# bioinfo-pf-curie/mpiBWA

Measured on AMD Instinct MI355X. Metric: Mreads/s (whole node) 2x150 bp PE vs GRCh38-size reference; SAM bit-match, higher is better.
Workload: dtype int32

## Files before the change

mpibwa_amd/csrc/aln_kernel.hip:

```cpp
#include <hip/hip_runtime.h>
#include <algorithm>
#include "device.h"
#include "wave_ext.cuh"

namespace mbw {

#define ALN_WAVES 1
__host__ __device__ inline int aln_zcap(int max_len) { int z = 80 * (max_len + 32); z = (z + 255) & ~255; return z < 12288 ? 12288 : z; }
__host__ __device__ inline int aln_zcap_small(int max_len) { int z = 32 * (max_len + 32); return (z + 255) & ~255; }
#define ALN_MDCAP 768
#define ALN_CIGCAP 96
#define ALN_NEG (-0x40000000)

__device__ __forceinline__ int wave_sum_int(int v)
{
	for (int o = 32; o > 0; o >>= 1) v += __shfl_xor(v, o);
	return v;
}

struct AlnLds {
	int *H, *E, *dummy;
	uint8_t *q, *t, *z, *md;
	uint32_t *cig;
};
#define ALN_PAD 64

__device__ __forceinline__ int put_num(uint8_t *md, int len, int v, int lane)
{
	char buf[12];
	int n = 0;
	if (v == 0) buf[n++] = '0';
	while (v > 0) { buf[n++] = '0' + v % 10; v /= 10; }
	if (lane == 0)
		for (int k = 0; k < n; ++k)
			if (len + k < ALN_MDCAP) md[len + k] = buf[n - 1 - k];
	return len + n;
}

#define ALN_PENDING 2
#define ALN_SLAB 1024u

__device__ __forceinline__ bool aln_invalid(const AlnParams &P, const AlnReq &R, int max_len, int tcap)
{
	const int lq = R.qe - R.qb;
	const long long rlen64 = R.re - R.rb;
	const bool bridging = R.rb < P.l_pac && R.re > P.l_pac;
	return lq <= 0 || rlen64 <= 0 || bridging || lq > max_len || rlen64 > tcap;
}
__device__ __forceinline__ bool aln_same_len(const AlnParams &P, const AlnReq &R, int max_len, int tcap)
{
	return !aln_invalid(P, R, max_len, tcap) && R.re - R.rb == R.qe - R.qb;
}

__global__ void __launch_bounds__(256) aln_classify_kernel(AlnParams P, int n_req, const AlnReq *__restrict__ reqs, int max_len, int tcap,
                                                           int *__restrict__ lists, unsigned long long *counters, int dp_kind)
{
	const int rq = blockIdx.x * 256 + threadIdx.x;
	const bool live = rq < n_req && reqs[rq < n_req ? rq : 0].read >= 0;
	bool nodp = false;
	if (live) nodp = aln_same_len(P, reqs[rq], max_len, tcap);
	const unsigned long long below = (1ull << (threadIdx.x & 63)) - 1;
	for (int pass = 0; pass < 2; ++pass) {
		const bool mine = live && (nodp == (pass == 0));
		const int kind = pass == 0 ? 0 : dp_kind;
		const unsigned long long m = __ballot(mine);
		if (!m) continue;
		unsigned long long base = 0;
		if ((threadIdx.x & 63) == __ffsll((long long)m) - 1) base = atomicAdd(&counters[ALN_CNT + kind], (unsigned long long)__popcll(m));
		base = __shfl(base, __ffsll((long long)m) - 1);
		if (mine) lists[(size_t)kind * n_req + base + __popcll(m & below)] = rq;
	}
}

template <int KIND>
__device__ __forceinline__ void aln_one(int rq, const AlnParams &P, const WxParams &X, int n_req, const AlnReq *__restrict__ reqs,
                                        const uint8_t *__restrict__ seq, const int64_t *__restrict__ off, const uint8_t *__restrict__ pac,
                                        const int *__restrict__ gaptab, AlnHdr *__restrict__ hdr, uint8_t *__restrict__ pool,
                                        unsigned long long *counters, unsigned long long pool_bytes, int max_len, int tcap, int *lists, int dp_kind,
                                        unsigned long long &slab_at, unsigned &slab_left)
{
	extern __shared__ int lds_raw[];
	const int wave = threadIdx.x >> 6, lane = threadIdx.x & 63;
	constexpr bool FAST = KIND == 0;
	const int ALN_ZCAP = KIND == 1 ? aln_zcap_small(max_len) : aln_zcap(max_len);
	AlnLds L;
	if (FAST) {
		const size_t per_wave = (size_t)2 * ((max_len + 3) & ~3) + ALN_MDCAP + 16;
		uint8_t *base = (uint8_t *)lds_raw + (size_t)wave * per_wave;
		L.H = L.E = L.dummy = nullptr; L.z = nullptr;
		L.cig = (uint32_t *)base;
		L.q = base + 16;
		L.t = L.q + ((max_len + 3) & ~3);
		L.md = L.t + ((max_len + 3) & ~3);
	} else {
		const size_t per_wave = (size_t)2 * (max_len + 2 + ALN_PAD) * 4 + 4 + ((max_len + 3) & ~3) + ((tcap + 3) & ~3) + ALN_ZCAP + ALN_MDCAP + ALN_CIGCAP * 4;
		uint8_t *base = (uint8_t *)lds_raw + (size_t)wave * per_wave;
		L.H = (int *)base; L.E = L.H + (max_len + 2 + ALN_PAD);
		L.dummy = L.E + (max_len + 2 + ALN_PAD);
		L.cig = (uint32_t *)(L.dummy + 1);
		L.q = (uint8_t *)(L.cig + ALN_CIGCAP);
		L.t = L.q + ((max_len + 3) & ~3);
		L.z = L.t + ((tcap + 3) & ~3);
		L.md = L.z + ALN_ZCAP;
	}

	AlnReq R = reqs[rq];
	if (KIND != 0) {
		const unsigned long long rb = (unsigned long long)R.rb, re = (unsigned long long)R.re;
		R.rb = (int64_t)((unsigned long long)(unsigned)__builtin_amdgcn_readfirstlane((int)(rb >> 32)) << 32 |
		                 (unsigned)__builtin_amdgcn_readfirstlane((int)rb));
		R.re = (int64_t)((unsigned long long)(unsigned)__builtin_amdgcn_readfirstlane((int)(re >> 32)) << 32 |
		                 (unsigned)__builtin_amdgcn_readfirstlane((int)re));
		R.read = __builtin_amdgcn_readfirstlane(R.read); R.qb = __builtin_amdgcn_readfirstlane(R.qb);
		R.qe = __builtin_amdgcn_readfirstlane(R.qe); R.w2 = __builtin_amdgcn_readfirstlane(R.w2);
		R.truesc = __builtin_amdgcn_readfirstlane(R.truesc);
	}
	const int lq = R.qe - R.qb;
	const long long rlen64 = R.re - R.rb;
	AlnHdr out;
	out.score = 0; out.NM = -1; out.n_cigar = 0; out.md_len = 0; out.pool_off = 0; out.flags = 0;
	const bool invalid = aln_invalid(P, R, max_len, tcap);
	if (invalid) {
		out.flags = 1;
		if (lane == 0) hdr[rq] = out;
		return;
	}
	const int rlen = (int)rlen64;
	const bool rev = R.rb >= P.l_pac;
	const uint8_t *rd = seq + off[R.read];
	for (int j = lane; j < lq; j += 64) L.q[j] = rev ? rd[R.qe - 1 - j] : rd[R.qb + j];
	{
		const long long f0 = rev ? (P.l_pac << 1) - R.re : R.rb;
		for (int i = lane; i < rlen; i += 64) {
			long long f = f0 + i;
			int b = (pac[f >> 2] >> ((~f & 3) << 1)) & 3;
			L.t[i] = rev ? 3 - b : b;
		}
	}
	__builtin_amdgcn_wave_barrier();

	const int oe_del = X.o_del + X.e_del, oe_ins = X.o_ins + X.e_ins, e_del = X.e_del, e_ins = X.e_ins;
	uint32_t plo[5], phi[5];
#pragma unroll
	for (int t = 0; t < 5; ++t) {
		plo[t] = (uint32_t)(uint8_t)X.mat[t * 5] | (uint32_t)(uint8_t)X.mat[t * 5 + 1] << 8 | (uint32_t)(uint8_t)X.mat[t * 5 + 2] << 16 |
		         (uint32_t)(uint8_t)X.mat[t * 5 + 3] << 24;
		phi[t] = (uint32_t)(uint8_t)X.mat[t * 5 + 4];
	}
	const int wmax4 = P.w << 2;
	int w2 = R.w2, last_sc = -(1 << 30), score = 0, n_cig = 0;
	bool fallback = false;
	for (int it = 0;; ) {
		w2 = w2 < wmax4 ? w2 : wmax4;
		if (FAST) {
			int s = 0;
			for (int i = lane; i < lq; i += 64) s += X.mat[L.t[i] * 5 + L.q[i]];
			score = wave_sum_int(s);
			if (w2 != 0) {
				int amax = X.mat[0];
				for (int k = 1; k < 25; ++k) amax = X.mat[k] > amax ? X.mat[k] : amax;
				if (amax <= 0 || (long long)lq * amax - score > (long long)amax + oe_del + oe_ins) {
					if (lane == 0) lists[(size_t)dp_kind * n_req + atomicAdd(&counters[ALN_CNT + dp_kind], 1ull)] = rq;
					return;
				}
			}
			n_cig = 1;
			if (lane == 0) L.cig[0] = (uint32_t)lq << 4;
			__builtin_amdgcn_fence(__ATOMIC_RELEASE, "wavefront");
			__builtin_amdgcn_wave_barrier();
			__builtin_amdgcn_fence(__ATOMIC_ACQUIRE, "wavefront");
			break;
		} else {
			int d_len = rlen - lq; d_len = d_len < 0 ? -d_len : d_len;
			int w = (gaptab[lq] + d_len + 1) >> 1;
			w = w < w2 ? w : w2;
			const int min_w = d_len + 3;
			w = w > min_w ? w : min_w;
			const int n_col = lq < 2 * w + 1 ? lq : 2 * w + 1;
			if ((long long)n_col * rlen > ALN_ZCAP) { fallback = true; break; }
			for (int j = lane; j <= lq; j += 64) {
				L.H[j] = j == 0 ? 0 : (j <= w ? -(X.o_ins + e_ins * j) : ALN_NEG);
				L.E[j] = ALN_NEG;
			}
			__builtin_amdgcn_wave_barrier();
			int vslo = 0, vshi = 0;
			for (int i = 0; i < rlen; ++i) {
				if ((i & 63) == 0) {
					const int tb = i + lane < rlen ? (int)L.t[i + lane] : 4;
					vslo = (int)(tb == 0 ? plo[0] : tb == 1 ? plo[1] : tb == 2 ? plo[2] : tb == 3 ? plo[3] : plo[4]);
					vshi = (int)(tb == 0 ? phi[0] : tb == 1 ? phi[1] : tb == 2 ? phi[2] : tb == 3 ? phi[3] : phi[4]);
				}
				const uint32_t slo = (uint32_t)__builtin_amdgcn_readlane(vslo, i & 63), shi = (uint32_t)__builtin_amdgcn_readlane(vshi, i & 63);
				const int beg = i > w ? i - w : 0, end = i + w + 1 < lq ? i + w + 1 : lq;
				const int hleft0 = beg == 0 ? -(X.o_del + e_del * (i + 1)) : ALN_NEG;
				const int n_row = end - beg;
				int A = ALN_NEG;
				int h_carry = hleft0;
				uint8_t *zi = L.z + (size_t)i * n_col;
				for (int s0 = 0; s0 <= n_row; s0 += 64) {
					const int j = beg + s0 + lane;
					const bool act = s0 + lane < n_row, wr = s0 + lane <= n_row;
					const int diag = L.H[j], e = L.E[j];
					const int qraw = (int)L.q[j];
					const int qb = act ? qraw : 4;
					const int sc = (int)(int8_t)__builtin_amdgcn_perm(shi, slo, (uint32_t)qb | 0x0c0c0c00u);
					const int m = diag + sc;
					const int g = act ? m - oe_ins + j * e_ins : ALN_NEG - (1 << 28);
					const int incl = wx_scan_max(g);
					const int excl = wx_dpp<0x138, 0xf>(ALN_NEG - (1 << 28), incl);
					const int f = max(A, excl + e_ins) - j * e_ins;
					uint8_t d = m >= e ? 0 : 1;
					int h = m >= e ? m : e;
					if (h < f) { d = 2; h = f; }
					int t = m - oe_del;
					int e2 = e - e_del;
					if (e2 > t) d |= 1 << 2; else e2 = t;
					t = m - oe_ins;
					if (f - e_ins > t) d |= 2 << 4;
					const int h_prev = wx_dpp<0x138, 0xf>(h_carry, h);
					(wr ? L.H + j : L.dummy)[0] = h_prev;
					(wr ? L.E + j : L.dummy)[0] = act ? e2 : ALN_NEG;
					(act ? zi + (j - beg) : (uint8_t *)L.dummy)[0] = d;
					A = max(A, __builtin_amdgcn_readlane(incl, 63) + e_ins);
					h_carry = __builtin_amdgcn_readlane(h, 63);
				}
				if (n_row < 0 && lane == 0) { L.H[end] = hleft0; L.E[end] = ALN_NEG; }
				__builtin_amdgcn_wave_barrier();
			}
			score = L.H[lq];
			{
				int which = 0, i = rlen - 1, k = (i + w + 1 < lq ? i + w + 1 : lq) - 1, n = 0;
				uint32_t cur = 0;
				bool ovf = false;
				auto push = [&](uint32_t op, uint32_t len) {
					if (cur && (cur & 0xf) == op) cur += len << 4;
					else {
						if (cur) { if (n < ALN_CIGCAP) { if (lane == 0) L.cig[n] = cur; } else ovf = true; ++n; }
						cur = len << 4 | op;
					}
				};
				while (i >= 0 && k >= 0) {
					which = __builtin_amdgcn_readfirstlane((int)L.z[(size_t)i * n_col + (k - (i > w ? i - w : 0))]) >> (which << 1) & 3;
					if (which == 0) { push(0, 1); --i; --k; }
					else if (which == 1) { push(2, 1); --i; }
					else { push(1, 1); --k; }
				}
				if (i >= 0) push(2, i + 1);
				if (k >= 0) push(1, k + 1);
				if (cur) { if (n < ALN_CIGCAP) { if (lane == 0) L.cig[n] = cur; } else ovf = true; ++n; }
				if (ovf) { fallback = true; break; }
				__builtin_amdgcn_wave_barrier();
				for (int a = lane; a < n / 2; a += 64) { uint32_t x = L.cig[a]; L.cig[a] = L.cig[n - 1 - a]; L.cig[n - 1 - a] = x; }
				__builtin_amdgcn_wave_barrier();
				n_cig = n;
			}
		}
		if (score == last_sc || w2 == wmax4) break;
		last_sc = score;
		w2 <<= 1;
		if (!(++it < 3 && score < R.truesc - P.a)) break;
	}
	if (fallback) {
		if (KIND == 1) {
			if (lane == 0) lists[(size_t)2 * n_req + atomicAdd(&counters[ALN_CNT + 2], 1ull)] = rq;
			return;
		}
		out.flags = 1;
		if (lane == 0) hdr[rq] = out;
		return;
	}
	int md_len = 0, n_mm = 0, n_gap = 0;
	{
		const char *int2base = rev ? "TGCAN" : "ACGTN";
		int x = 0, y = 0, u = 0;
		for (int k = 0; k < n_cig; ++k) {
			const uint32_t c = L.cig[k];
			const int op = c & 0xf, len = (int)(c >> 4);
			if (op == 0) {
				for (int i0 = 0; i0 < len; i0 += 64) {
					const int i = i0 + lane;
					unsigned long long mm = __ballot(i < len && L.q[x + i] != L.t[y + i]);
					int cur = 0;
					const int chunk = len - i0 < 64 ? len - i0 : 64;
					while (mm) {
						const int p = __ffsll((long long)mm) - 1;
						mm &= mm - 1;
						u += p - cur;
						md_len = put_num(L.md, md_len, u, lane);
						if (lane == 0 && md_len < ALN_MDCAP) L.md[md_len] = int2base[L.t[y + i0 + p]];
						++md_len; ++n_mm; u = 0; cur = p + 1;
					}
					u += chunk - cur;
				}
				x += len; y += len;
			} else if (op == 2) {
				if (k > 0 && k < n_cig - 1) {
					md_len = put_num(L.md, md_len, u, lane);
					if (lane == 0 && md_len < ALN_MDCAP) L.md[md_len] = '^';
					++md_len;
					for (int i = lane; i < len; i += 64)
						if (md_len + i < ALN_MDCAP) L.md[md_len + i] = int2base[L.t[y + i]];
					md_len += len;
					u = 0; n_gap += len;
				}
				y += len;
			} else { x += len; n_gap += len; }
		}
		md_len = put_num(L.md, md_len, u, lane);
	}
	if (md_len > ALN_MDCAP) {
		out.flags = 1;
		if (lane == 0) hdr[rq] = out;
		return;
	}
	__builtin_amdgcn_wave_barrier();
	const unsigned need = (unsigned)n_cig * 4 + (((unsigned)md_len + 3) & ~3u);
	unsigned long long at = 0;
	if (need <= slab_left) { at = slab_at; slab_at += need; slab_left -= need; }
	else {
		const unsigned take = need > ALN_SLAB ? need : ALN_SLAB;
		if (lane == 0) at = atomicAdd(&counters[0], (unsigned long long)take);
		at = __shfl(at, 0);
		slab_at = at + need; slab_left = take - need;
	}
	if (at + need > pool_bytes) {
		out.flags = 1;
		if (lane == 0) hdr[rq] = out;
		return;
	}
	uint32_t *pc = (uint32_t *)(pool + at);
	for (int k = lane; k < n_cig; k += 64) pc[k] = L.cig[k];
	uint8_t *pm = pool + at + (size_t)n_cig * 4;
	for (int k = lane; k < md_len; k += 64) pm[k] = L.md[k];
	out.score = score; out.NM = n_mm + n_gap; out.n_cigar = n_cig; out.md_len = md_len; out.pool_off = (uint32_t)(at >> 2); out.flags = 0;
	if (lane == 0) hdr[rq] = out;
}

template <int KIND>
__global__ void __launch_bounds__(64 * ALN_WAVES)
aln_kernel(AlnParams P, WxParams X, int n_req, const AlnReq *__restrict__ reqs, const uint8_t *__restrict__ seq,
           const int64_t *__restrict__ off, const uint8_t *__restrict__ pac, const int *__restrict__ gaptab, AlnHdr *__restrict__ hdr,
           uint8_t *__restrict__ pool, unsigned long long *counters, unsigned long long pool_bytes, int max_len, int tcap, int *lists, int dp_kind)
{
	const int wave = threadIdx.x >> 6;
	const int n = (int)counters[ALN_CNT + KIND];
	const int *mine = lists + (size_t)KIND * n_req;
	unsigned long long slab_at = 0;
	unsigned slab_left = 0;
	for (int k = blockIdx.x * ALN_WAVES + wave; k < n; k += gridDim.x * ALN_WAVES) {
		aln_one<KIND>(KIND != 0 ? __builtin_amdgcn_readfirstlane(mine[k]) : mine[k], P, X, n_req, reqs, seq, off, pac, gaptab, hdr, pool, counters, pool_bytes, max_len, tcap, lists, dp_kind,
		              slab_at, slab_left);
		__builtin_amdgcn_fence(__ATOMIC_RELEASE, "wavefront");
		__builtin_amdgcn_wave_barrier();
		__builtin_amdgcn_fence(__ATOMIC_ACQUIRE, "wavefront");
	}
}

size_t aln_lds_per_block(int max_len, int tcap)
{
	const int ALN_ZCAP = aln_zcap(max_len);
	size_t per_wave = (size_t)2 * (max_len + 2 + ALN_PAD) * 4 + 4 + ((max_len + 3) & ~3) + ((tcap + 3) & ~3) + ALN_ZCAP + ALN_MDCAP + ALN_CIGCAP * 4;
	return per_wave * ALN_WAVES;
}

void launch_aln(void *stream, const AlnParams &P, const ExtParams &ep, int n_req, const AlnReq *d_req, const uint8_t *d_seq,
                const int64_t *d_off, const uint8_t *d_pac, const int *d_gaptab, AlnHdr *d_hdr, uint8_t *d_pool,
                unsigned long long *d_counters, size_t pool_bytes, int max_len, int tcap, int *d_lists, bool wide_only)
{
	if (n_req <= 0) return;
	const WxParams X = wx_params(ep);
	const size_t shmem = aln_lds_per_block(max_len, tcap);
	const size_t shmem_small = shmem - (size_t)(aln_zcap(max_len) - aln_zcap_small(max_len)) * ALN_WAVES;
	const size_t shmem_fast = ((size_t)2 * ((max_len + 3) & ~3) + ALN_MDCAP + 16) * ALN_WAVES;
	if (shmem > 64 * 1024 && hipFuncSetAttribute((const void *)aln_kernel<2>, hipFuncAttributeMaxDynamicSharedMemorySize, (int)shmem) != hipSuccess)
		die("aln_kernel: cannot reserve %zu bytes of LDS", shmem);
	if (shmem_small > 64 * 1024 && hipFuncSetAttribute((const void *)aln_kernel<1>, hipFuncAttributeMaxDynamicSharedMemorySize, (int)shmem_small) != hipSuccess)
		die("aln_kernel: cannot reserve %zu bytes of LDS", shmem_small);
	if (shmem_fast > 64 * 1024) die("aln_kernel: reads of %d bp do not fit the LDS staging buffers", max_len);
	static int s_cus = 0;
	if (!s_cus) {
		int dev = 0;
		hipDeviceProp_t prop;
		if (hipGetDevice(&dev) != hipSuccess || hipGetDeviceProperties(&prop, dev) != hipSuccess) die("aln_kernel: cannot query the device");
		s_cus = prop.multiProcessorCount > 0 ? prop.multiProcessorCount : 256;
	}
	auto grid_for = [&](size_t lds) {
		long long per_cu = (long long)(160 * 1024 / std::max<size_t>(lds, 1));
		per_cu = std::max(1ll, std::min(per_cu, 32ll / ALN_WAVES));
		return dim3((unsigned)std::min<long long>((long long)s_cus * per_cu * 2, ((long long)n_req + ALN_WAVES - 1) / ALN_WAVES));
	};
	const dim3 block(64 * ALN_WAVES);
	hipStream_t st = (hipStream_t)stream;
	hipLaunchKernelGGL(aln_classify_kernel, dim3((n_req + 255) / 256), dim3(256), 0, st, P, n_req, d_req, max_len, tcap, d_lists, d_counters,
	                   wide_only ? 2 : 1);
	hipLaunchKernelGGL(aln_kernel<0>, grid_for(shmem_fast), block, shmem_fast, st, P, X, n_req, d_req, d_seq, d_off, d_pac, d_gaptab, d_hdr, d_pool,
	                   d_counters, (unsigned long long)pool_bytes, max_len, tcap, d_lists, wide_only ? 2 : 1);
	hipLaunchKernelGGL(aln_kernel<1>, grid_for(shmem_small), block, shmem_small, st, P, X, n_req, d_req, d_seq, d_off, d_pac, d_gaptab, d_hdr, d_pool,
	                   d_counters, (unsigned long long)pool_bytes, max_len, tcap, d_lists, wide_only ? 2 : 1);
	hipLaunchKernelGGL(aln_kernel<2>, grid_for(shmem), block, shmem, st, P, X, n_req, d_req, d_seq, d_off, d_pac, d_gaptab, d_hdr, d_pool,
	                   d_counters, (unsigned long long)pool_bytes, max_len, tcap, d_lists, wide_only ? 2 : 1);
	if (hipGetLastError() != hipSuccess) die("aln_kernel: launch failed");
}

}
```

mpibwa_amd/csrc/device.h:

```cpp
#ifndef MBW_DEVICE_H
#define MBW_DEVICE_H
#include "internal.h"
#include <mutex>
#include <vector>

namespace mbw {

struct FmDev {
	const void *blk;
	const void *occ32;
	const void *occ_sb;
	const uint64_t *sa;
	const uint64_t *sa_full;
	uint64_t primary, seq_len;
	uint64_t L2[5];
	int sa_shift;
	const void *p3tab;
	int p3_k;
	const void *kmt;
	int kmt_k;
};

struct DevIndex {
	int device = -1;
// ... 82 lines not shown
struct DevReg {
	int64_t rb, re;
	int32_t qb, qe, rid, score, truesc, w, seedcov, seedlen0;
	float frac_rep;
	int32_t pad;
};
struct C2aParams {
	int64_t l_pac;
	int a, w, pen_clip5, pen_clip3;
	int early;
};
struct C2aUnits {
	int max_units = 0, heavy_t = 0;
	const unsigned int *n_units = nullptr;
	const int *ustart = nullptr;
	const int *unit_rd = nullptr, *unit_av = nullptr;
	const int *clist = nullptr;
	int *c_rabs = nullptr, *c_rcnt = nullptr;
};
struct C2aGroupBufs {
	PinBuf h_heavy, h_hoff, h_nunits;
	DevBuf heavy, hoff, scratch, clist, ustart, unit_rd, unit_av, nunits, c_rabs, c_rcnt;
	void release()
	{
		for (PinBuf *b : {&h_heavy, &h_hoff, &h_nunits}) b->release();
		for (DevBuf *b : {&heavy, &hoff, &scratch, &clist, &ustart, &unit_rd, &unit_av, &nunits, &c_rabs, &c_rcnt}) b->release();
	}
};
C2aUnits c2a_prepare_units(void *stream, C2aGroupBufs &B, int heavy_t, int n, const int *chain_cnt, size_t n_chain_slots, const int *d_chain_beg,
                           const int *d_reg_beg, const DevChain *d_chains, int *d_nregs, void (*wait)(void *stream) = nullptr);
void c2a_launch_order(int n, const int *nseeds, int *order);
void c2a_length_tables(const mem_opt_t *opt, int max_len, std::vector<int> &tab);
void c2a_params(const mem_opt_t *opt, int64_t l_pac, int early, C2aParams &cp, ExtParams &ep);
size_t c2a_groups_scratch_bytes(int n_el);
void launch_c2a_groups(void *stream, int n_el, int n_heavy, const int *d_hoff, const int *d_heavy, const int *d_chain_beg, const int *d_reg_beg,
                       const DevChain *d_chains, void *d_scratch, int *d_clist, int *d_ustart, int *d_unit_rd, int *d_unit_av, unsigned int *d_n_units);
#define C2A_STAT_SLOTS 256
void launch_c2a(void *stream, const C2aParams &P, const ExtParams &ep, int n_reads, const uint8_t *d_seq, const int64_t *d_off,
                const int *d_len, const int *d_chain_beg, const int *d_chain_cnt, const DevChain *d_chains, const DevSeed *d_seeds, unsigned int *d_srt,
                const int *d_reg_beg, DevReg *d_regs, int *d_nregs, const int *d_tab, int tab_stride, const uint8_t *d_pac, unsigned long long *d_counters,
                int max_len, const int *d_order = nullptr, const C2aUnits *units = nullptr );

struct ChainParams {
	int64_t l_pac;
	int w, max_chain_gap, min_chain_weight, min_seed_len, max_chain_extend;
	float mask_level, drop_ratio;
};
ChainParams chain_params(const mem_opt_t *opt, int64_t l_pac);
void contig_table(const bntseq_t *bns, std::vector<int64_t> &ann_off, std::vector<uint8_t> &ann_alt);
void launch_chain(void *stream, const ChainParams &P, int n_reads, const int *d_len, const int *d_nseeds, const int *d_lrep,
                  const int64_t *d_seed_off, const uint64_t *d_sa, const int32_t *d_qbl, const int64_t *d_ann_off, const uint8_t *d_ann_alt,
                  int n_seqs, const int *d_tab, int tab_stride, DevChain *d_chains, DevSeed *d_seeds, unsigned int *d_srt, int *d_nchains,
                  void *d_scratch);
size_t chain_scratch_bytes(int n_reads);

size_t reg_pack_tmp_bytes(int n_reads);
void launch_reg_pack(void *stream, int n_reads, const int *d_reg_beg, const int *d_nregs, int *d_reg_pos, const DevReg *d_regs, DevReg *d_packed,
                     void *d_tmp, size_t tmp_bytes, const C2aUnits *units = nullptr, const int *d_chain_beg = nullptr, const int *d_chain_cnt = nullptr);
struct C2aJob {
	int n_reads = 0, max_len = 0;
	const uint8_t *d_seq = nullptr; const int64_t *d_off = nullptr; const int *d_len = nullptr;
	const int *d_chain_beg = nullptr, *d_chain_cnt = nullptr, *d_reg_beg = nullptr, *d_order = nullptr;
	const DevChain *d_chains = nullptr; const DevSeed *d_seeds = nullptr; unsigned int *d_srt = nullptr;
	const int *d_tab = nullptr; int tab_stride = 0;
	const uint8_t *d_pac = nullptr;
	C2aUnits units;
	DevReg *d_regs = nullptr; int *d_nregs = nullptr;
	unsigned long long *d_stat = nullptr;
	int *d_reg_pos = nullptr; DevReg *d_packed = nullptr; void *d_tmp = nullptr; size_t tmp_bytes = 0;
};
void queue_c2a(void *stream, const mem_opt_t *opt, int64_t l_pac, int early, const C2aJob &J, void *ev_a = nullptr, void *ev_b = nullptr);

struct AlnReq {
	int64_t rb, re;
	int32_t read, qb, qe, w2, truesc, pad;
};
struct AlnHdr {
	int32_t score, NM, n_cigar, md_len;
	uint32_t pool_off;
	int32_t flags;
};
struct AlnParams { int64_t l_pac; int a, w; };
#define ALN_CNT 8
void aln_params(const mem_opt_t *opt, int64_t l_pac, AlnParams &ap, ExtParams &ep);
inline size_t aln_pool_bytes(size_t n_req) { return n_req * 96 + ((size_t)48 << 20); }
void cigar_gap_table(const mem_opt_t *opt, int max_len, std::vector<int> &tab);
size_t aln_lds_per_block(int max_len, int tcap);
void launch_aln(void *stream, const AlnParams &P, const ExtParams &ep, int n_req, const AlnReq *d_req, const uint8_t *d_seq,
                const int64_t *d_off, const uint8_t *d_pac, const int *d_gaptab, AlnHdr *d_hdr, uint8_t *d_pool,
                unsigned long long *d_counters, size_t pool_bytes, int max_len, int tcap, int *d_lists ,
                bool wide_only = false );

struct SamDesc {
	int64_t rb, re;
	int32_t qb, qe;
	int32_t req;
	int32_t rid, flag, mapq, score, sub;
};
#define SAM_XA_SHIFT 16
#define SAM_XA_MASK 15
struct SamParams {
	int64_t l_pac;
	int has_qual, rg_len;
	char rg[256];
};
SamParams sam_params(int64_t l_pac, bool has_qual);
void contig_names(const bntseq_t *bns, std::vector<char> &names, std::vector<int> &name_off);
size_t sam_arena_bytes(int n_reads, int max_len);
struct ChunkDev {
	const uint8_t *d_seq = nullptr; const int64_t *d_off = nullptr; const int *d_len = nullptr; int max_len = 0;
	const uint8_t *d_pac = nullptr; const int *d_gap = nullptr;
	const uint8_t *d_qual = nullptr, *d_names = nullptr; const int *d_noff = nullptr;
	const int64_t *d_ann_off = nullptr; const uint8_t *d_ann_alt = nullptr; const char *d_ann_names = nullptr; const int *d_ann_noff = nullptr;
};
struct AlnSamJob {
	int n_req = 0; const AlnReq *d_req = nullptr; AlnHdr *d_hdr = nullptr; uint8_t *d_pool = nullptr; size_t pool_bytes = 0;
	unsigned long long *d_cnt = nullptr; int *d_lists = nullptr;
	int ends = 2, r0 = 0, n_reads = 0;
	const SamDesc *h_desc = nullptr;
	SamDesc *d_desc = nullptr;
	const int *h_base = nullptr; int *d_base = nullptr;
	uint8_t *d_arena = nullptr; size_t arena_bytes = 0; unsigned long long *d_used = nullptr, *d_ooff = nullptr; int *d_olen = nullptr;
	int grid_blocks = 0;
	int n_multi = 0; const int *d_mlist = nullptr; const uint8_t *d_mlines = nullptr; const SamDesc *d_mdesc = nullptr; const int *d_mbase = nullptr;
};
void queue_aln_sam(void *stream, const mem_opt_t *opt, int64_t l_pac, const ChunkDev &D, const SamParams &sp, const AlnSamJob &J,
                   void *ev_a = nullptr, void *ev_b = nullptr);
void launch_sam_emit(void *stream, const SamParams &P, int n_reads, const SamDesc *d_desc, const int *d_req_base, const AlnReq *d_req, const AlnHdr *d_hdr,
                     const uint8_t *d_pool, const uint8_t *d_seq, const int64_t *d_off, const int *d_len, const uint8_t *d_qual,
                     const uint8_t *d_names, const int *d_name_off, const int64_t *d_ann_off, const char *d_ann_names, const int *d_ann_name_off,
                     uint8_t *d_arena, size_t arena_bytes, unsigned long long *d_arena_used, unsigned long long *d_out_off, int *d_out_len,
                     int grid_blocks = 0);
void launch_sam_emit_se(void *stream, const SamParams &P, int n_reads, const SamDesc *d_desc, const int *d_req_base, const AlnReq *d_req, const AlnHdr *d_hdr,
                        const uint8_t *d_pool, const uint8_t *d_seq, const int64_t *d_off, const int *d_len, const uint8_t *d_qual,
                        const uint8_t *d_names, const int *d_name_off, const int64_t *d_ann_off, const char *d_ann_names, const int *d_ann_name_off,
                        uint8_t *d_arena, size_t arena_bytes, unsigned long long *d_arena_used, unsigned long long *d_out_off, int *d_out_len,
                        int grid_blocks = 0);
void launch_sam_lines(void *stream, const SamParams &P, bool softclip, int n_units, const int *d_list, int r0, const uint8_t *d_n_lines, const SamDesc *d_ldesc,
                      const int *d_req_base, const AlnReq *d_req, const AlnHdr *d_hdr, const uint8_t *d_pool, const uint8_t *d_seq, const int64_t *d_off,
                      const int *d_len, const uint8_t *d_qual, const uint8_t *d_names, const int *d_name_off, const int64_t *d_ann_off,
                      const char *d_ann_names, const int *d_ann_name_off, uint8_t *d_arena, size_t arena_bytes, unsigned long long *d_arena_used,
                      unsigned long long *d_out_off, int *d_out_len, int grid_blocks = 0, bool pe = false);
int sam_lines_row(void);
int sam_lines_sa_stage(void);

struct MswReq;
struct MswRes;
#define PR_MAXREG 8
extern "C" int mi355x_pair_maxreg(void);
struct PairParams {
	int64_t l_pac;
	int a, b, pen_unpaired, min_seed_len, w, o_del, e_del, o_ins, e_ins, max_chain_gap, T, max_matesw;
	float mask_level_redun, mask_level, XA_drop_ratio;
	uint64_t id0;
	int lnq[64];
	int no_rescue;
	int low[4], high[4], failed[4];
	int tab_off[4];
	int ltab_n;
	int max_XA_hits;
};
bool pair_params(const mem_opt_t *opt, int64_t l_pac, const mem_pestat_t pes[4], int64_t n_processed, int max_len, PairParams &P, size_t *n_tab);
void pair_tables(const mem_opt_t *opt, const mem_pestat_t pes[4], const PairParams &P, size_t n_tab, double *tab);
void launch_first_reg(void *stream, int n, const int *d_reg_pos, const int *d_nregs, const DevReg *d_packed, DevReg *d_first, int *d_nfirst);
#define PR_HOST 0
#define PR_DECIDED 1
// ... 145 lines not shown
```

mpibwa_amd/csrc/sam_stage.hip:

```cpp
#include "pipeline.h"

namespace mbw {

static_assert(sizeof(SamDesc) == sizeof(SamDescH), "host/device record layouts differ");
static_assert(sizeof(MswReq) == sizeof(MswReqH) && sizeof(MswRes) == sizeof(MswResH), "host/device record layouts differ");
static_assert(sizeof(AlnReq) == sizeof(AlnReqH) && sizeof(AlnHdr) == sizeof(AlnHdrH), "host/device record layouts differ");
static const int MSW_MAX_T = 4096;

void Call::start_sam_inputs()
{
	gpu_aln = getenv("MPIBWA_HOST_CIGAR") == nullptr && aln_lds_per_block(max_len, max_len + 256) <= (size_t)160 * 1024;
	se_want = !pe && gpu_aln && getenv("MPIBWA_HOST_SAM") == nullptr && getenv("MPIBWA_HOST_SE") == nullptr && opt->mapQ_coef_len > 0 &&
	          !(opt->flag & (MEM_F_ALL | MEM_F_REF_HDR | MEM_F_PRIMARY5));
	sam_inputs.t = std::thread([this] { sam_inputs_body(); });
}

void Call::sam_inputs_body()
{
	HIP_OK(hipSetDevice(ix.device));
	hipStream_t sst = C.d_streams[1];
	std::vector<int> gaptab;
	cigar_gap_table(opt, max_len, gaptab);
	int *d_gap = (int *)W.agap.ensure(gaptab.size() * 4);
	D.d_gap = d_gap;
// ... 439 lines not shown
		}
		if (cpusec_on()) { tsc_plan += tsc_plan_blk; tsc_emitc += tsc_emitc_blk; }
	});
	if (round == 1) {
		P.base.assign(nu + 1, 0);
		for (int i = 0; i < nu; ++i) P.base[i + 1] = P.base[i] + P.u_cnt[i];
		P.n_req = P.base[nu];
		P.req = (AlnReqH *)W.h_areq[P.slot].ensure(P.n_req * sizeof(AlnReqH) + 64);
		parallel_for(n_thr, nu, 4096, [&](int i) {
			if (P.u_cnt[i]) memcpy(&P.req[P.base[i]], &P.blk_req[i >> 8][P.u_first[i]], (size_t)P.u_cnt[i] * sizeof(AlnReqH));
		});
	}
	plan_ms += now_ms() - ta;
	cpu_collect += cpu_sec() - ca;
}

void Call::job_launch(Job &J, JobBufs &B, hipStream_t jst, const Part &P, const AlnReq *d_req, size_t n_req, const uint32_t *base, bool with_sam,
                      const SamDescH *h_desc, SamDesc *d_desc, const WaveBufs *multi, int n_multi)
{
	const int ends = pe ? 2 : 1;
	const int nu = P.hi - P.lo, nr = nu * ends;
	J.B = &B; J.st = jst; J.n_req = n_req; J.n_reads = nr;
	J.pool_bytes = aln_pool_bytes(n_req);
	AlnSamJob Q;
	AlnReq *d_up = d_req ? nullptr : (AlnReq *)B.req.ensure(n_req * sizeof(AlnReq));
	J.d_hdr = (AlnHdr *)B.hdr.ensure(n_req * sizeof(AlnHdr));
	J.d_pool = (uint8_t *)B.pool.ensure(J.pool_bytes);
	J.d_cnt = (unsigned long long *)B.cnt.ensure(256);
	if (d_up) HIP_OK(hipMemcpyAsync(d_up, P.req, n_req * sizeof(AlnReq), hipMemcpyHostToDevice, jst));
	Q.n_req = (int)n_req; Q.d_req = d_req ? d_req : d_up; Q.d_hdr = J.d_hdr; Q.d_pool = J.d_pool; Q.pool_bytes = J.pool_bytes; Q.d_cnt = J.d_cnt;
	Q.d_lists = (int *)B.lists.ensure(n_req * 3 * sizeof(int));
	if (with_sam) {
		int *hb = (int *)B.h_base.ensure((size_t)(nu + 1) * 4 + 64);
		for (int k = 0; k <= nu; ++k) hb[k] = base ? (int)base[k] : ends * k;
		J.arena_bytes = sam_arena_bytes(nr, max_len);
		Q.ends = ends; Q.r0 = P.lo * ends; Q.n_reads = nr;
		Q.h_desc = (const SamDesc *)h_desc; Q.d_desc = d_desc;
		Q.h_base = hb; Q.d_base = (int *)B.base.ensure((size_t)(nu + 1) * 4);
		Q.d_arena = (uint8_t *)B.arena.ensure(J.arena_bytes); Q.arena_bytes = J.arena_bytes;
		Q.d_used = (unsigned long long *)B.used.ensure(64);
		Q.d_ooff = (unsigned long long *)B.ooff.ensure((size_t)nr * 8);
		Q.d_olen = (int *)B.olen.ensure((size_t)nr * 4);
		if (multi && n_multi > 0) {
			const int s = P.slot;
			Q.n_multi = n_multi; Q.d_mlist = (const int *)multi->work.p; Q.d_mlines = (const uint8_t *)multi->nlines.p;
			Q.d_mdesc = (const SamDesc *)multi->ldesc.p; Q.d_mbase = (const int *)W.wave[s].ldst.p;
		}
	}
	queue_aln_sam(jst, opt, bns->l_pac, D, sam_par, Q, J.ev.a, J.ev.b);
	J.launched = true; J.sam_launched = with_sam;
}

static void fetch_results(Job &J)
{
	JobBufs &B = *J.B;
	HIP_OK(hipMemcpyAsync(J.small_cnt, J.d_cnt, 64, hipMemcpyDeviceToHost, J.st));
	stream_wait(J.st);
	const size_t used = std::min<size_t>(J.small_cnt[0], J.pool_bytes);
	AlnHdrH *hh = (AlnHdrH *)B.h_hdr.ensure(J.n_req * sizeof(AlnHdr) + 64);
	uint8_t *hp = (uint8_t *)B.h_pool.ensure(used + 64);
	HIP_OK(hipMemcpyAsync(hh, J.d_hdr, J.n_req * sizeof(AlnHdr), hipMemcpyDeviceToHost, J.st));
	if (used) HIP_OK(hipMemcpyAsync(hp, J.d_pool, used, hipMemcpyDeviceToHost, J.st));
	stream_wait(J.st);
	J.hdr = hh; J.pool = hp;
}

static void fetch_records(Job &J)
{
	JobBufs &B = *J.B;
	const int nr = J.n_reads;
	HIP_OK(hipMemcpyAsync(J.small_used, B.used.p, 8, hipMemcpyDeviceToHost, J.st));
	stream_wait(J.st);
	const unsigned long long used = std::min<unsigned long long>(J.small_used[0], J.arena_bytes);
	uint8_t *ha = (uint8_t *)B.h_arena.ensure((size_t)used + 64);
	unsigned long long *ho = (unsigned long long *)B.h_ooff.ensure((size_t)nr * 8 + 64);
	int *hl = (int *)B.h_olen.ensure((size_t)nr * 4 + 64);
	if (used) HIP_OK(hipMemcpyAsync(ha, B.arena.p, (size_t)used, hipMemcpyDeviceToHost, J.st));
	HIP_OK(hipMemcpyAsync(ho, B.ooff.p, (size_t)nr * 8, hipMemcpyDeviceToHost, J.st));
	HIP_OK(hipMemcpyAsync(hl, B.olen.p, (size_t)nr * 4, hipMemcpyDeviceToHost, J.st));
	stream_wait(J.st);
	J.sarena = ha; J.sooff = ho; J.solen = hl;
}

void Call::job_fetch(Job &J, const Part &P, Fetch policy, bool wave_units)
{
	if (!J.launched) return;
	const double ta = now_ms();
	stream_wait(J.st);
	HIP_OK(hipGetLastError());
	STAT.k_aln_ms += J.ev.ms();
	STAT.n_aln += J.n_req;
	if (policy == FETCH_ALWAYS) fetch_results(J);
	if (J.sam_launched) fetch_records(J);
	if (policy == FETCH_IF_HANDED_BACK) {
		const int ends = pe ? 2 : 1;
		bool any_back = false;
		for (int k = 0; k < P.hi - P.lo && !any_back; ++k)
			for (int e = 0; e < ends; ++e)
				any_back = any_back || (ustat[P.lo + k] == PR_DECIDED && (!wave_units || wave_dec[P.lo + k]) && !(dev_se_wave && wave_dec[P.lo + k]) &&
				                        J.solen[ends * k + e] < 0);
		if (any_back) fetch_results(J);
	}
	aln_wait_ms += now_ms() - ta;
}

void Call::launch_dev(Part &P)
{
	stage(14);
	if (!dev_units || !d_pr_req || P.hi == P.lo) return;
	const int ends = pe ? 2 : 1;
	unsigned long long *small = (unsigned long long *)W.h_small[P.slot].ensure(512);
	P.dev.small_used = small; P.dev.small_cnt = small + 8;
	job_launch(P.dev, W.dev_job[P.slot], C.d_streams[P.slot], P, d_pr_req + (size_t)P.lo * ends, (size_t)(P.hi - P.lo) * ends, nullptr, true, nullptr,
	           const_cast<SamDesc *>(d_pr_desc));
}
void Call::finish_dev(Part &P)
{
	stage(15);
	job_fetch(P.dev, P, FETCH_IF_HANDED_BACK);
}
void Call::launch(Part &P)
{
	stage(16);
	if (!gpu_aln || P.n_req == 0) return;
	unsigned long long *small = (unsigned long long *)W.h_small[P.slot].ensure(512);
	P.host.small_cnt = small + 16; P.host.small_used = small + 24;
	SamDesc *d_desc = gpu_sam ? (SamDesc *)W.sdesc.ensure((size_t)n * sizeof(SamDesc)) : nullptr;
	job_launch(P.host, W.host_job[P.slot], C.a_streams[P.slot], P, nullptr, P.n_req, P.base.data(), gpu_sam, sdesc, d_desc);
}
void Call::finish(Part &P)
{
	stage(17);
	job_fetch(P.host, P, FETCH_ALWAYS);
	if (cpusec_on() && P.host.launched) {
		unsigned long long c[16];
		HIP_OK(hipMemcpy(c, P.host.d_cnt, sizeof c, hipMemcpyDeviceToHost));
		fprintf(stderr, "[aln lists] %zu requests: same-length %llu, narrow DP %llu, full DP %llu\n", P.host.n_req, c[8], c[9], c[10]);
	}
}

void Call::take_record(int read, const Job &J, int at)
{
	const int len = J.solen[at];
	char *sam = (char *)malloc((size_t)len + 1);
	if (!sam) die("out of memory");
	memcpy(sam, J.sarena + J.sooff[at], (size_t)len);
	sam[len] = 0;
	seqs[read].sam = sam;
}

void Call::replay(Part &P, int which)
{
	stage(18);
	const double ta = now_ms(), ca = cpu_sec(), sa_ = sys_sec();
	const long pf = page_faults();
	const int ends = pe ? 2 : 1;
	if (pe || which != 0 || dev_units) parallel_blocks(n_thr, P.hi - P.lo, pe ? 128 : 256, [&](int, int, int k_lo, int k_hi) {
		unsigned long long n_dev = 0, n_se_xa_w = 0, n_se_supp_w = 0, n_pair_lines_w = 0, tsc = 0;
		for (int k = k_lo; k < k_hi; ++k) {
			const int i = P.lo + k, r = ends * i;
			const bool lines_k = pe && dev_units && ustat[i] == PW_DECIDED_LINES;
			const bool xa_k = (dev_units && ustat[i] == PW_DECIDED_XA) || lines_k || (dev_se_wave && wave_dec[i]);
			const bool dev_k = xa_k || (dev_units && ustat[i] == PR_DECIDED);
			const bool own_k = xa_k || (dev_k && P.wave.launched && wave_dec[i]);
			const Job &J = xa_k ? P.xa : own_k ? P.wave : dev_k ? P.dev : P.host;
			bool written = J.solen != nullptr;
			for (int e = 0; e < ends && written; ++e) written = J.solen[ends * k + e] >= 0;
			const bool early = dev_k && written && !own_k;
			if (which != 2 && early != (which == 0)) continue;
			if (written) {
				const unsigned long long tq0 = cpusec_on() ? __builtin_ia32_rdtsc() : 0;
				for (int e = 0; e < ends; ++e) take_record(r + e, J, ends * k + e);
				if (!pe && ustat[i] == SE_DECIDED_XA) ++n_se_xa_w;
				else if (!pe && ustat[i] == SE_DECIDED_LINES) ++n_se_supp_w;
				else if (lines_k) ++n_pair_lines_w;
				else n_dev += ends;
				if (cpusec_on()) tsc += __builtin_ia32_rdtsc() - tq0;
				continue;
			}
			AlnCtx ctx;
			if (gpu_aln) { ctx.mode = AlnCtx::REPLAY; ctx.hdr = P.host.hdr; ctx.pool = P.host.pool; ctx.cursor = P.base[k]; }
			if (dev_k) { ctx.hdr = J.hdr; ctx.pool = J.pool; ctx.cursor = (size_t)ends * k; }
			if (pe) {
				MswCtx mc;
				const bool has_msw = dev_k && dev_wave && (wave_dec[i] || xa_k) && P.msw_launched && P.mbase[k + 1] != P.mbase[k];
				if (has_msw) { mc.req = P.mreq + P.mbase[k]; mc.res = P.mres + P.mbase[k]; mc.n = (int)(P.mbase[k + 1] - P.mbase[k]); }
				if (dev_k) sam_pe_plan(opt, bns, pac, pes, (uint64_t)((n_processed >> 1) + i), &seqs[r], &regs[r], plans[i], has_msw ? &mc : nullptr, r);
				sam_pe_emit(opt, bns, pac, pes, &seqs[r], &regs[r], plans[i], gpu_aln && !xa_k ? &ctx : nullptr, r);
			} else {
				if (dev_k) mark_primary_se(opt, regs[i], n_processed + i);
				reg2sam(opt, bns, pac, &seqs[i], regs[i], 0, 0, gpu_aln && !xa_k ? &ctx : nullptr, i);
			}
		}
		n_sam_dev += n_dev; n_se_xa_sam += n_se_xa_w; n_se_supp_sam += n_se_supp_w; n_pair_lines_sam += n_pair_lines_w; tsc_devcopy += tsc;
	});
	emit_ms += now_ms() - ta;
	cpu_emit += cpu_sec() - ca;
	sys_emit += sys_sec() - sa_; pf_emit += page_faults() - pf;
}

void Call::sam_stage()
{
	n_units = pe ? n >> 1 : n;
	plans.resize(pe ? n_units : 0);
	n_parts = (gpu_aln && n_units >= 20000 && n_sub > 1) ? 2 : 1;
	if (const char *e = getenv("MPIBWA_SAM_PARTS")) n_parts = std::max(1, std::min(2, atoi(e)));
	gpu_msw = pe && !(opt->flag & MEM_F_NO_RESCUE) && getenv("MPIBWA_HOST_MATESW") == nullptr && (int64_t)max_len * opt->a < 8192 &&
	          msw_lds_bytes(max_len) <= 160 * 1024 && msw_on_device(opt);
	const char *dle = getenv("MPIBWA_DEV_JOB_LATE");
	const bool dev_late = dle ? atoi(dle) != 0 : crowded;
	const bool dev_early = pe && !dev_late, dev_mid = !pe, dev_last = pe && dev_late;
	dev_wave = pe && dev_units && gpu_msw && getenv("MPIBWA_HOST_RESCUE") == nullptr;
	if (dev_wave) { wave_cand.assign(n_units, 0); wave_dec.assign(n_units, 0); }
	dev_xa = dev_wave && gpu_sam && wave_pp.max_XA_hits <= PW_XA_CAP && getenv("MPIBWA_HOST_XA") == nullptr;
	const char *hpl = getenv("MPIBWA_HOST_PAIR_LINES");
	dev_pair_lines = dev_wave && gpu_sam && !(hpl && atoi(hpl) != 0);
	for (int p = 0; p < n_parts; ++p) {
		parts[p].slot = p;
		parts[p].lo = p ? n_units / 2 : 0;
		parts[p].hi = p == n_parts - 1 ? n_units : n_units / 2;
	}
// ... 60 lines not shown
```

Measured before the change: 7.965.

## Alias DP LDS scratch buffers, batch diagonal traceback, and set occupancy bounds

Shrinks per-wave LDS for the DP kernels by aliasing the CIGAR buffer onto H and the MD buffer onto the traceback matrix, with wavefront fences at the hand-overs, so more waves fit per CU. Traceback now scans up to 64 diagonal steps at once with a ballot instead of one readfirstlane per step. Launch bounds now request a per-kind minimum waves per SIMD, put_num is rewritten without a local buffer, and an env-gated clock64 profiling path is added. Aliasing risks data hazards if the ordering is wrong, and the tighter launch bounds may cause register spills.

```diff
diff --git a/mpibwa_amd/csrc/aln_kernel.hip b/mpibwa_amd/csrc/aln_kernel.hip
--- a/mpibwa_amd/csrc/aln_kernel.hip
+++ b/mpibwa_amd/csrc/aln_kernel.hip
@@ -24,22 +24,38 @@
 	uint32_t *cig;
 };
 #define ALN_PAD 64
+__host__ __device__ inline size_t aln_lds_dp(int max_len, int tcap, int zcap)
+{
+	return (size_t)2 * (max_len + 2 + ALN_PAD) * 4 + 4 + ((max_len + 3) & ~3) + ((tcap + 3) & ~3) + zcap;
+}
+__device__ __forceinline__ void aln_lds_handover()
+{
+	__builtin_amdgcn_fence(__ATOMIC_RELEASE, "wavefront");
+	__builtin_amdgcn_wave_barrier();
+	__builtin_amdgcn_fence(__ATOMIC_ACQUIRE, "wavefront");
+}
 
 __device__ __forceinline__ int put_num(uint8_t *md, int len, int v, int lane)
 {
-	char buf[12];
-	int n = 0;
-	if (v == 0) buf[n++] = '0';
-	while (v > 0) { buf[n++] = '0' + v % 10; v /= 10; }
+	int n = 1;
+	for (unsigned p = 10; (unsigned)v >= p && n < 10; p *= 10) ++n;
 	if (lane == 0)
-		for (int k = 0; k < n; ++k)
-			if (len + k < ALN_MDCAP) md[len + k] = buf[n - 1 - k];
+		for (int k = n - 1; k >= 0; --k, v /= 10)
+			if (len + k < ALN_MDCAP) md[len + k] = '0' + v % 10;
 	return len + n;
 }
 
-#define ALN_PENDING 2
 #define ALN_SLAB 1024u
 
+__device__ __forceinline__ int aln_band(const int *__restrict__ gaptab, int lq, int rlen, int w2, int &w)
+{
+	int d_len = rlen - lq; d_len = d_len < 0 ? -d_len : d_len;
+	w = (gaptab[lq] + d_len + 1) >> 1;
+	w = w < w2 ? w : w2;
+	const int min_w = d_len + 3;
+	w = w > min_w ? w : min_w;
+	return lq < 2 * w + 1 ? lq : 2 * w + 1;
+}
 __device__ __forceinline__ bool aln_invalid(const AlnParams &P, const AlnReq &R, int max_len, int tcap)
 {
 	const int lq = R.qe - R.qb;
@@ -72,7 +88,9 @@
 	}
 }
 
-template <int KIND>
+__device__ __forceinline__ int aln_zcol(int i, int k, int w) { return k - (i > w ? i - w : 0); }
+
+template <int KIND, bool PROF>
 __device__ __forceinline__ void aln_one(int rq, const AlnParams &P, const WxParams &X, int n_req, const AlnReq *__restrict__ reqs,
                                         const uint8_t *__restrict__ seq, const int64_t *__restrict__ off, const uint8_t *__restrict__ pac,
                                         const int *__restrict__ gaptab, AlnHdr *__restrict__ hdr, uint8_t *__restrict__ pool,
@@ -81,6 +99,14 @@
 {
 	extern __shared__ int lds_raw[];
 	const int wave = threadIdx.x >> 6, lane = threadIdx.x & 63;
+	unsigned long long t_prof = PROF ? (unsigned long long)clock64() : 0;
+	auto lap = [&](int phase) {
+		if (PROF) {
+			const unsigned long long now = (unsigned long long)clock64();
+			if (lane == 0) atomicAdd(&counters[ALN_PROF_AT + 4 * (KIND - 1) + phase], now - t_prof);
+			t_prof = now;
+		}
+	};
 	constexpr bool FAST = KIND == 0;
 	const int ALN_ZCAP = KIND == 1 ? aln_zcap_small(max_len) : aln_zcap(max_len);
 	AlnLds L;
@@ -93,15 +119,14 @@
 		L.t = L.q + ((max_len + 3) & ~3);
 		L.md = L.t + ((max_len + 3) & ~3);
 	} else {
-		const size_t per_wave = (size_t)2 * (max_len + 2 + ALN_PAD) * 4 + 4 + ((max_len + 3) & ~3) + ((tcap + 3) & ~3) + ALN_ZCAP + ALN_MDCAP + ALN_CIGCAP * 4;
-		uint8_t *base = (uint8_t *)lds_raw + (size_t)wave * per_wave;
+		uint8_t *base = (uint8_t *)lds_raw + (size_t)wave * aln_lds_dp(max_len, tcap, ALN_ZCAP);
 		L.H = (int *)base; L.E = L.H + (max_len + 2 + ALN_PAD);
 		L.dummy = L.E + (max_len + 2 + ALN_PAD);
-		L.cig = (uint32_t *)(L.dummy + 1);
-		L.q = (uint8_t *)(L.cig + ALN_CIGCAP);
+		L.cig = (uint32_t *)L.H;
+		L.q = (uint8_t *)(L.dummy + 1);
 		L.t = L.q + ((max_len + 3) & ~3);
 		L.z = L.t + ((tcap + 3) & ~3);
-		L.md = L.z + ALN_ZCAP;
+		L.md = L.z;
 	}
 
 	AlnReq R = reqs[rq];
@@ -128,9 +153,11 @@
 	const int rlen = (int)rlen64;
 	const bool rev = R.rb >= P.l_pac;
 	const uint8_t *rd = seq + off[R.read];
+#pragma unroll 2
 	for (int j = lane; j < lq; j += 64) L.q[j] = rev ? rd[R.qe - 1 - j] : rd[R.qb + j];
 	{
 		const long long f0 = rev ? (P.l_pac << 1) - R.re : R.rb;
+#pragma unroll 2
 		for (int i = lane; i < rlen; i += 64) {
 			long long f = f0 + i;
 			int b = (pac[f >> 2] >> ((~f & 3) << 1)) & 3;
@@ -138,6 +165,7 @@
 		}
 	}
 	__builtin_amdgcn_wave_barrier();
+	if (!FAST) lap(0);
 
 	const int oe_del = X.o_del + X.e_del, oe_ins = X.o_ins + X.e_ins, e_del = X.e_del, e_ins = X.e_ins;
 	uint32_t plo[5], phi[5];
@@ -171,13 +199,15 @@
 			__builtin_amdgcn_fence(__ATOMIC_ACQUIRE, "wavefront");
 			break;
 		} else {
-			int d_len = rlen - lq; d_len = d_len < 0 ? -d_len : d_len;
-			int w = (gaptab[lq] + d_len + 1) >> 1;
-			w = w < w2 ? w : w2;
-			const int min_w = d_len + 3;
-			w = w > min_w ? w : min_w;
-			const int n_col = lq < 2 * w + 1 ? lq : 2 * w + 1;
+			int w;
+			const int n_col = aln_band(gaptab, lq, rlen, w2, w);
+			if (PROF && it == 0 && lane == 0 && KIND == dp_kind) {
+				const long long area = (long long)n_col * rlen;
+				atomicAdd(&counters[ALN_PROF_NCOL + (n_col <= 7 ? 0 : n_col <= 9 ? 1 : n_col <= 11 ? 2 : n_col <= 16 ? 3 : n_col <= 21 ? 4 : n_col <= 32 ? 5 : 6)], 1ull);
+				atomicAdd(&counters[ALN_PROF_AREA + (area <= aln_zcap_small(max_len) / 2 ? 0 : area <= aln_zcap_small(max_len) ? 1 : 2)], 1ull);
+			}
 			if ((long long)n_col * rlen > ALN_ZCAP) { fallback = true; break; }
+#pragma unroll 1
 			for (int j = lane; j <= lq; j += 64) {
 				L.H[j] = j == 0 ? 0 : (j <= w ? -(X.o_ins + e_ins * j) : ALN_NEG);
 				L.E[j] = ALN_NEG;
@@ -227,7 +257,9 @@
 				if (n_row < 0 && lane == 0) { L.H[end] = hleft0; L.E[end] = ALN_NEG; }
 				__builtin_amdgcn_wave_barrier();
 			}
-			score = L.H[lq];
+			score = __builtin_amdgcn_readfirstlane(L.H[lq]);
+			aln_lds_handover();
+			lap(1);
 			{
 				int which = 0, i = rlen - 1, k = (i + w + 1 < lq ? i + w + 1 : lq) - 1, n = 0;
 				uint32_t cur = 0;
@@ -240,7 +272,16 @@
 					}
 				};
 				while (i >= 0 && k >= 0) {
-					which = __builtin_amdgcn_readfirstlane((int)L.z[(size_t)i * n_col + (k - (i > w ? i - w : 0))]) >> (which << 1) & 3;
+					if (which == 0) {
+						const int ii = i - lane, kk = k - lane;
+						const bool in = ii >= 0 && kk >= 0;
+						const int d = in ? (int)L.z[(size_t)ii * n_col + aln_zcol(ii, kk, w)] : 0;
+						const unsigned long long stop = __ballot(!in || (d & 3) != 0);
+						const int run = stop ? __ffsll((long long)stop) - 1 : 64;
+						if (run) { push(0, (uint32_t)run); i -= run; k -= run; }
+						if (run == 64 || i < 0 || k < 0) continue;
+					}
+					which = __builtin_amdgcn_readfirstlane((int)L.z[(size_t)i * n_col + aln_zcol(i, k, w)]) >> (which << 1) & 3;
 					if (which == 0) { push(0, 1); --i; --k; }
 					else if (which == 1) { push(2, 1); --i; }
 					else { push(1, 1); --k; }
@@ -249,11 +290,12 @@
 				if (k >= 0) push(1, k + 1);
 				if (cur) { if (n < ALN_CIGCAP) { if (lane == 0) L.cig[n] = cur; } else ovf = true; ++n; }
 				if (ovf) { fallback = true; break; }
-				__builtin_amdgcn_wave_barrier();
+				aln_lds_handover();
 				for (int a = lane; a < n / 2; a += 64) { uint32_t x = L.cig[a]; L.cig[a] = L.cig[n - 1 - a]; L.cig[n - 1 - a] = x; }
-				__builtin_amdgcn_wave_barrier();
+				aln_lds_handover();
 				n_cig = n;
 			}
+			lap(2);
 		}
 		if (score == last_sc || w2 == wmax4) break;
 		last_sc = score;
@@ -269,6 +311,7 @@
 		if (lane == 0) hdr[rq] = out;
 		return;
 	}
+	if (!FAST) aln_lds_handover();
 	int md_len = 0, n_mm = 0, n_gap = 0;
 	{
 		const char *int2base = rev ? "TGCAN" : "ACGTN";
@@ -329,15 +372,20 @@
 		return;
 	}
 	uint32_t *pc = (uint32_t *)(pool + at);
+#pragma unroll 1
 	for (int k = lane; k < n_cig; k += 64) pc[k] = L.cig[k];
 	uint8_t *pm = pool + at + (size_t)n_cig * 4;
+#pragma clang loop unroll(disable) vectorize(disable) interleave(disable)
 	for (int k = lane; k < md_len; k += 64) pm[k] = L.md[k];
 	out.score = score; out.NM = n_mm + n_gap; out.n_cigar = n_cig; out.md_len = md_len; out.pool_off = (uint32_t)(at >> 2); out.flags = 0;
 	if (lane == 0) hdr[rq] = out;
-}
-
-template <int KIND>
-__global__ void __launch_bounds__(64 * ALN_WAVES)
+	if (!FAST) lap(3);
+}
+
+__host__ __device__ constexpr int aln_waves_per_simd(int kind) { return kind == 0 ? 6 : kind == 1 ? 5 : 2; }
+
+template <int KIND, bool PROF>
+__global__ void __launch_bounds__(64 * ALN_WAVES, aln_waves_per_simd(KIND))
 aln_kernel(AlnParams P, WxParams X, int n_req, const AlnReq *__restrict__ reqs, const uint8_t *__restrict__ seq,
            const int64_t *__restrict__ off, const uint8_t *__restrict__ pac, const int *__restrict__ gaptab, AlnHdr *__restrict__ hdr,
            uint8_t *__restrict__ pool, unsigned long long *counters, unsigned long long pool_bytes, int max_len, int tcap, int *lists, int dp_kind)
@@ -348,19 +396,15 @@
 	unsigned long long slab_at = 0;
 	unsigned slab_left = 0;
 	for (int k = blockIdx.x * ALN_WAVES + wave; k < n; k += gridDim.x * ALN_WAVES) {
-		aln_one<KIND>(KIND != 0 ? __builtin_amdgcn_readfirstlane(mine[k]) : mine[k], P, X, n_req, reqs, seq, off, pac, gaptab, hdr, pool, counters, pool_bytes, max_len, tcap, lists, dp_kind,
-		              slab_at, slab_left);
-		__builtin_amdgcn_fence(__ATOMIC_RELEASE, "wavefront");
-		__builtin_amdgcn_wave_barrier();
-		__builtin_amdgcn_fence(__ATOMIC_ACQUIRE, "wavefront");
+		aln_one<KIND, PROF>(KIND != 0 ? __builtin_amdgcn_readfirstlane(mine[k]) : mine[k], P, X, n_req, reqs, seq, off, pac, gaptab, hdr, pool, counters, pool_bytes, max_len, tcap, lists,
+		                    dp_kind, slab_at, slab_left);
+		aln_lds_handover();
 	}
 }
 
 size_t aln_lds_per_block(int max_len, int tcap)
 {
-	const int ALN_ZCAP = aln_zcap(max_len);
-	size_t per_wave = (size_t)2 * (max_len + 2 + ALN_PAD) * 4 + 4 + ((max_len + 3) & ~3) + ((tcap + 3) & ~3) + ALN_ZCAP + ALN_MDCAP + ALN_CIGCAP * 4;
-	return per_wave * ALN_WAVES;
+	return aln_lds_dp(max_len, tcap, aln_zcap(max_len)) * ALN_WAVES;
 }
 
 void launch_aln(void *stream, const AlnParams &P, const ExtParams &ep, int n_req, const AlnReq *d_req, const uint8_t *d_seq,
@@ -370,12 +414,8 @@
 	if (n_req <= 0) return;
 	const WxParams X = wx_params(ep);
 	const size_t shmem = aln_lds_per_block(max_len, tcap);
-	const size_t shmem_small = shmem - (size_t)(aln_zcap(max_len) - aln_zcap_small(max_len)) * ALN_WAVES;
+	const size_t shmem_small = aln_lds_dp(max_len, tcap, aln_zcap_small(max_len)) * ALN_WAVES;
 	const size_t shmem_fast = ((size_t)2 * ((max_len + 3) & ~3) + ALN_MDCAP + 16) * ALN_WAVES;
-	if (shmem > 64 * 1024 && hipFuncSetAttribute((const void *)aln_kernel<2>, hipFuncAttributeMaxDynamicSharedMemorySize, (int)shmem) != hipSuccess)
-		die("aln_kernel: cannot reserve %zu bytes of LDS", shmem);
-	if (shmem_small > 64 * 1024 && hipFuncSetAttribute((const void *)aln_kernel<1>, hipFuncAttributeMaxDynamicSharedMemorySize, (int)shmem_small) != hipSuccess)
-		die("aln_kernel: cannot reserve %zu bytes of LDS", shmem_small);
 	if (shmem_fast > 64 * 1024) die("aln_kernel: reads of %d bp do not fit the LDS staging buffers", max_len);
 	static int s_cus = 0;
 	if (!s_cus) {
@@ -391,14 +431,18 @@
 	};
 	const dim3 block(64 * ALN_WAVES);
 	hipStream_t st = (hipStream_t)stream;
-	hipLaunchKernelGGL(aln_classify_kernel, dim3((n_req + 255) / 256), dim3(256), 0, st, P, n_req, d_req, max_len, tcap, d_lists, d_counters,
-	                   wide_only ? 2 : 1);
-	hipLaunchKernelGGL(aln_kernel<0>, grid_for(shmem_fast), block, shmem_fast, st, P, X, n_req, d_req, d_seq, d_off, d_pac, d_gaptab, d_hdr, d_pool,
-	                   d_counters, (unsigned long long)pool_bytes, max_len, tcap, d_lists, wide_only ? 2 : 1);
-	hipLaunchKernelGGL(aln_kernel<1>, grid_for(shmem_small), block, shmem_small, st, P, X, n_req, d_req, d_seq, d_off, d_pac, d_gaptab, d_hdr, d_pool,
-	                   d_counters, (unsigned long long)pool_bytes, max_len, tcap, d_lists, wide_only ? 2 : 1);
-	hipLaunchKernelGGL(aln_kernel<2>, grid_for(shmem), block, shmem, st, P, X, n_req, d_req, d_seq, d_off, d_pac, d_gaptab, d_hdr, d_pool,
-	                   d_counters, (unsigned long long)pool_bytes, max_len, tcap, d_lists, wide_only ? 2 : 1);
+	const int dp_kind = wide_only ? 2 : 1;
+	hipLaunchKernelGGL(aln_classify_kernel, dim3((n_req + 255) / 256), dim3(256), 0, st, P, n_req, d_req, max_len, tcap, d_lists, d_counters, dp_kind);
+	auto run = [&](auto kernel, size_t lds) {
+		if (lds > 64 * 1024 && hipFuncSetAttribute((const void *)kernel, hipFuncAttributeMaxDynamicSharedMemorySize, (int)lds) != hipSuccess)
+			die("aln_kernel: cannot reserve %zu bytes of LDS", lds);
+		hipLaunchKernelGGL(kernel, grid_for(lds), block, lds, st, P, X, n_req, d_req, d_seq, d_off, d_pac, d_gaptab, d_hdr, d_pool, d_counters,
+		                   (unsigned long long)pool_bytes, max_len, tcap, d_lists, dp_kind);
+	};
+	const bool prof = getenv("MPIBWA_ALN_PROF") && atoi(getenv("MPIBWA_ALN_PROF")) != 0;
+	run(aln_kernel<0, false>, shmem_fast);
+	if (prof) { run(aln_kernel<1, true>, shmem_small); run(aln_kernel<2, true>, shmem); }
+	else { run(aln_kernel<1, false>, shmem_small); run(aln_kernel<2, false>, shmem); }
 	if (hipGetLastError() != hipSuccess) die("aln_kernel: launch failed");
 }
 
diff --git a/mpibwa_amd/csrc/device.h b/mpibwa_amd/csrc/device.h
--- a/mpibwa_amd/csrc/device.h
+++ b/mpibwa_amd/csrc/device.h
@@ -188,6 +188,9 @@
 };
 struct AlnParams { int64_t l_pac; int a, w; };
 #define ALN_CNT 8
+#define ALN_PROF_AT 16
+#define ALN_PROF_NCOL 1
+#define ALN_PROF_AREA 28
 void aln_params(const mem_opt_t *opt, int64_t l_pac, AlnParams &ap, ExtParams &ep);
 inline size_t aln_pool_bytes(size_t n_req) { return n_req * 96 + ((size_t)48 << 20); }
 void cigar_gap_table(const mem_opt_t *opt, int max_len, std::vector<int> &tab);
diff --git a/mpibwa_amd/csrc/sam_stage.hip b/mpibwa_amd/csrc/sam_stage.hip
--- a/mpibwa_amd/csrc/sam_stage.hip
+++ b/mpibwa_amd/csrc/sam_stage.hip
@@ -545,6 +545,24 @@
 	J.sarena = ha; J.sooff = ho; J.solen = hl;
 }
 
+static void print_aln_lists(const char *what, const Job &J)
+{
+	if (!cpusec_on() || !J.launched || !J.n_req) return;
+	unsigned long long c[32];
+	HIP_OK(hipMemcpy(c, J.d_cnt, sizeof c, hipMemcpyDeviceToHost));
+	fprintf(stderr, "[aln lists] %s job, %zu requests: same-length %llu, narrow DP %llu, full DP %llu\n", what, J.n_req, c[ALN_CNT], c[ALN_CNT + 1], c[ALN_CNT + 2]);
+	if (getenv("MPIBWA_ALN_PROF") && atoi(getenv("MPIBWA_ALN_PROF")) != 0) {
+		for (int kind = 1; kind <= 2; ++kind) {
+			const unsigned long long *t = c + ALN_PROF_AT + 4 * (kind - 1);
+			fprintf(stderr, "[aln prof] kind %d (%s): ticks of lane 0 in staging %llu, DP rows %llu, traceback %llu, MD + hand-over %llu\n", kind,
+			        kind == 1 ? "narrow" : "full size", t[0], t[1], t[2], t[3]);
+		}
+		const unsigned long long *h = c + ALN_PROF_NCOL, *a = c + ALN_PROF_AREA;
+		fprintf(stderr, "[aln prof] first rounds of the DP list: n_col <= 7: %llu, <= 9: %llu, <= 11: %llu, <= 16: %llu, <= 21: %llu, <= 32: %llu, above: %llu; "
+		        "n_col * rlen <= half the narrow matrix: %llu, <= the narrow matrix: %llu, above: %llu\n", h[0], h[1], h[2], h[3], h[4], h[5], h[6], a[0], a[1], a[2]);
+	}
+}
+
 void Call::job_fetch(Job &J, const Part &P, Fetch policy, bool wave_units)
 {
 	if (!J.launched) return;
@@ -581,6 +599,7 @@
 {
 	stage(15);
 	job_fetch(P.dev, P, FETCH_IF_HANDED_BACK);
+	print_aln_lists("device", P.dev);
 }
 void Call::launch(Part &P)
 {
@@ -595,11 +614,7 @@
 {
 	stage(17);
 	job_fetch(P.host, P, FETCH_ALWAYS);
-	if (cpusec_on() && P.host.launched) {
-		unsigned long long c[16];
-		HIP_OK(hipMemcpy(c, P.host.d_cnt, sizeof c, hipMemcpyDeviceToHost));
-		fprintf(stderr, "[aln lists] %zu requests: same-length %llu, narrow DP %llu, full DP %llu\n", P.host.n_req, c[8], c[9], c[10]);
-	}
+	print_aln_lists("host", P.host);
 }
 
 void Call::take_record(int read, const Job &J, int at)
```

Result: faster. 8.148 (median of 5 runs) (+2.3%).
